# arancormonk/dsd-neo

Hardware: AMD Instinct MI355X
Metric: I/Q Msamples/s end-to-end (demod->FEC->MBE) per GPU; % HBM roofline (higher is better)
Workload: dtype f32

## Files before the change

### dsd-neo_amd/csrc/ddn_api_chain.cpp

```cpp
#include <hip/hip_runtime.h>
#include <hsa/hsa.h>
#include <hsa/hsa_ext_amd.h>

#include <condition_variable>
#include <cstdio>
#include <cstdlib>
#include <cstring>
#include <deque>
#include <mutex>
#include <new>
#include <thread>

#include "ddn_api_util.h"
#include "ddn_chain.h"
#include "ddn_device.h"
#include "ddn_hip.h"
#include "ddn_internal.h"
#include "ddn_mbe.h"

enum { NSET = 3 };
static inline int
set_prev(int cur) {
    return (cur + NSET - 1) % NSET;
}
// ... 666 lines not shown
        {
            std::unique_lock<std::mutex> lk(*c->out_mu);
            c->out_cv->wait(lk, [&] { return c->out_stop || !c->out_q->empty(); });
            if (c->out_stop) {
                return;
            }
            job = c->out_q->front();
            c->out_q->pop_front();
        }
        int rc = DDN_OK;
        if (hipEventSynchronize(c->ev_consumed[job.set]) != hipSuccess) {
            rc = DDN_EHIP;
        } else {
            rc = chain_copy_out(c, &job.out, job.set);
        }
        {
            std::lock_guard<std::mutex> lk(*c->out_mu);
            if (rc != DDN_OK && c->out_rc == DDN_OK) {
                c->out_rc = rc;
                snprintf(c->out_err, sizeof(c->out_err), "%s", ddn_last_error());
            }
            c->out_issued[job.set]++;
        }
        c->out_cv->notify_all();
    }
}

static int
out_worker_start(ddn_p25_chain* c) {
    if (c->out_thread) {
        return DDN_OK;
    }
    HIP_TRY(hipGetDevice(&c->out_dev));
    c->out_mu = new (std::nothrow) std::mutex();
    c->out_cv = new (std::nothrow) std::condition_variable();
    c->out_q = new (std::nothrow) std::deque<ddn_p25_chain::OutJob>();
    if (!c->out_mu || !c->out_cv || !c->out_q) {
        return DDN_ENOMEM;
    }
    c->out_thread = new (std::nothrow) std::thread(out_worker, c);
    return c->out_thread ? DDN_OK : DDN_ENOMEM;
}

static int
chain_issue_pending(ddn_p25_chain* c, hipEvent_t beside) {
    if (!c->have_pending) {
        return DDN_OK;
    }
    const int set = c->pending_set;
    if (c->sdma > 0) {
        DDN_TRY(out_worker_start(c));
        c->have_pending = 0;
        {
            std::lock_guard<std::mutex> lk(*c->out_mu);
            ddn_p25_chain::OutJob job;
            job.set = set;
            job.out = c->pending_out;
            c->out_q->push_back(job);
            c->out_submitted[set]++;
        }
        c->out_cv->notify_all();
        return out_take_rc(c);
    }
    HIP_TRY(hipStreamWaitEvent(c->s_copy2, c->ev_consumed[set], 0));
    if (beside) {
        HIP_TRY(hipStreamWaitEvent(c->s_copy2, beside, 0));
    }
    DDN_TRY(chain_copy_out(c, &c->pending_out, set));
    HIP_TRY(hipEventRecord(c->ev_out[set], c->s_copy2));
    c->have_pending = 0;
    return DDN_OK;
}

static int chain_issue_deferred(ddn_p25_chain* c, hipEvent_t gate);

static int
chain_settle_pending(ddn_p25_chain* c, hipStream_t st, bool deferred_too = true) {
    if (c->have_deferred && deferred_too) {
        const int set = c->deferred_set;
        DDN_TRY(chain_issue_deferred(c, nullptr));
        HIP_TRY(hipStreamWaitEvent(st, c->ev_consumed[set], 0));
    }
    if (!c->have_pending) {
        return DDN_OK;
    }
    const int set = c->pending_set;
    DDN_TRY(chain_issue_pending(c, nullptr));
    if (c->sdma > 0) {
        for (int k = 0; k < NSET; k++) {
            sdma_wait(c, k);
        }
        return DDN_OK;
    }
    HIP_TRY(hipStreamWaitEvent(st, c->ev_out[set], 0));
    return DDN_OK;
}

static int
chain_long_pdu(ddn_p25_chain* c, int cur, int flush, hipStream_t st) {
    const DdnLongPdu* lp = &c->lp;
    const int NW = lp->B * lp->W;
    const int32_t *d_ns = nullptr, *d_sp = nullptr;
    DDN_TRY(ddn_p25p1_framer_device_syncs(c->fr, &d_ns, &d_sp));
    HIP_TRY(ddn_dev_lpdu_index(lp, c->d_evl[cur], c->d_evdl[cur], c->d_nevl[cur], c->EL, d_sp, d_ns, c->d_nid[cur], c->d_cnt_full[cur],
                               c->stride, c->d_new[set_prev(cur)], c->step > 0 ? 1 : 0, flush, c->F, c->T, c->off97[0], st));
    HIP_TRY(ddn_dev_lpdu_gather(lp, c->d_rec[cur], c->d_cnt_full[cur], c->stride, st));
    HIP_TRY(ddn_dev_p25_half_rate_list_wanted_wide(lp->wk_llr, NW, 8, lp->wk_want, (uint32_t*)lp->wk_cand, lp->wk_cnt, st));
    HIP_TRY(ddn_dev_chain_pdu_take_first(lp->wk_cand, lp->wk_cnt, NW, lp->wk_b12, lp->wk_metric, st));
    DDN_TRY(ddn_fec_p25_mbf34_list_batch(lp->wk_llr, (size_t)NW, 8, lp->wk_want34, (ddn_p25_mbf34_candidate*)lp->wk_cand, lp->wk_cnt, st));
    HIP_TRY(ddn_dev_chain_pdu_r34_select(lp->wk_cand, lp->wk_cnt, lp->wk_want34, NW, lp->wk_b18, lp->wk_c9, st));
    HIP_TRY(ddn_dev_lpdu_scatter(lp, st));
    HIP_TRY(ddn_dev_lpdu_finish(lp, st));
    return DDN_OK;
}

static int
chain_decode(ddn_p25_chain* c, int cur, int flush, hipStream_t st, hipEvent_t ev_pre = nullptr, bool defer_synth = false) {
    const size_t S = c->S, V = c->V, stride = c->stride;
    const uint8_t* rec = c->d_rec[cur];
    if (c->timing) {
        HIP_TRY(hipEventRecord(c->ev_t[3], st));
    }
    HIP_TRY(ddn_dev_chain_counts(c->d_new[cur], c->T, c->B, flush, c->d_cnt_scan, c->d_cnt_full[cur], st));
    DDN_TRY(ddn_p25p1_framer_index(c->fr, c->d_fl[cur], c->d_cnt_scan, stride, st));
    {
        const int prev = set_prev(cur);
        HIP_TRY(ddn_dev_chain_events(c->d_evl[prev], c->d_evdl[prev], c->d_nevl[prev], c->d_new[prev], c->step > 0 ? 1 : 0, c->d_ev[cur],
                                     c->d_evd[cur], c->d_nev[cur], c->E, c->EL, c->T, c->B, c->d_evl[cur], c->d_evdl[cur], c->d_nevl[cur],
                                     st));
        const int32_t *d_ns = nullptr, *d_sp = nullptr;
        DDN_TRY(ddn_p25p1_framer_device_syncs(c->fr, &d_ns, &d_sp));
        HIP_TRY(ddn_dev_zero_words(c->d_list_n, 8, st));
        HIP_TRY(ddn_dev_chain_frames(c->d_evl[cur], c->d_evdl[cur], c->d_nevl[cur], c->EL, d_sp, d_ns, c->B, c->F, c->off97[0],
                                     c->off97[1], c->off97[2], c->d_nid[cur], c->d_tsbk[cur], c->d_tsbk_crc, c->d_cls, c->d_lists, c->d_list_n,
                                     st));
    }
    hipStream_t vst = st;
    if (!c->timing && st == c->s_aux) {
        HIP_TRY(hipEventRecord(c->ev_fork, st));
        HIP_TRY(hipStreamWaitEvent(c->s_voice, c->ev_fork, 0));
        vst = c->s_voice;
    }
    struct SelGuard {
        ~SelGuard() { ddn_sel_clear(); }
    } sel_guard;
    for (int i = 0; i < 2; i++) {
        const int ldu = i + 1;
        ddn_sel_set(c->d_lists + (size_t)i * S, c->d_list_n + i);
        DDN_TRY(ddn_p25p1_framer_gather_ldu_words(c->fr, ldu, rec, c->d_cnt_full[cur], stride, c->d_words[i], c->d_wrel, c->d_vldu, st));
        DDN_TRY(ddn_fec_hamming_10_6_3_batch(c->d_words[i], S * 24, c->d_werrs, st));
        DDN_TRY(ddn_p25p1_framer_pack_ldu_rs(c->fr, ldu, c->d_words[i], c->d_rs_d[i], c->d_rs_p[i], st));
        DDN_TRY(ddn_fec_p25_rs_batch(i == 0 ? DDN_RS_24_12_13 : DDN_RS_24_16_9, c->d_rs_d[i], c->d_rs_p[i], S, c->d_rs_st[i], st));
    }
    ddn_sel_set(c->d_lists + (size_t)DDN_LIST_HDU * S, c->d_list_n + DDN_LIST_HDU);
    DDN_TRY(ddn_p25p1_framer_gather_hdu(c->fr, rec, c->d_cnt_full[cur], stride, c->d_hdu_hex, c->d_hdu_par, nullptr, nullptr, c->d_vldu, st));
    DDN_TRY(ddn_fec_golay24_batch(6, c->d_hdu_hex, c->d_hdu_par, S * 36, c->d_hdu_st, nullptr, st));
    DDN_TRY(ddn_p25p1_framer_pack_hdu_rs(c->fr, c->d_hdu_hex, c->d_hdu_d, c->d_hdu_p, st));
    DDN_TRY(ddn_fec_p25_rs_batch(DDN_RS_36_20_17, c->d_hdu_d, c->d_hdu_p, S, c->d_hdu_rs, st));
    ddn_sel_set(c->d_lists + (size_t)DDN_LIST_TDULC * S, c->d_list_n + DDN_LIST_TDULC);
    DDN_TRY(ddn_p25p1_framer_gather_tdulc(c->fr, rec, c->d_cnt_full[cur], stride, c->d_td_d, c->d_td_p, nullptr, nullptr, c->d_vldu, st));
    DDN_TRY(ddn_fec_golay24_batch(12, c->d_td_d, c->d_td_p, S * 12, c->d_td_st, nullptr, st));
    DDN_TRY(ddn_p25p1_framer_pack_tdulc_rs(c->fr, c->d_td_d, c->d_td_rd, c->d_td_rp, st));
    DDN_TRY(ddn_fec_p25_rs_batch(DDN_RS_24_12_13, c->d_td_rd, c->d_td_rp, S, c->d_td_rs, st));
    ddn_sel_set(c->d_lists + (size_t)DDN_LIST_LSD * S, c->d_list_n + DDN_LIST_LSD);
    DDN_TRY(ddn_p25p1_framer_gather_lsd(c->fr, rec, c->d_cnt_full[cur], stride, c->d_lsd, c->d_lsd_llr, c->d_vldu, st));
    DDN_TRY(ddn_fec_p25_lsd_batch(c->d_lsd, c->d_lsd_llr, S * 2, c->d_lsd_ok, st));
    ddn_sel_clear();
    {
        const int32_t *d_ns = nullptr, *d_sp = nullptr;
        DDN_TRY(ddn_p25p1_framer_device_syncs(c->fr, &d_ns, &d_sp));
        const size_t NE = (size_t)c->B * (size_t)c->PF, NB = NE * (size_t)c->PB;
        HIP_TRY(ddn_dev_chain_pdu_index(c->d_evl[cur], c->d_evdl[cur], c->d_nevl[cur], c->EL, d_sp, d_ns, c->d_nid[cur], c->B, c->F, c->off97[0],
                                        c->PF, c->d_pdu_slot, c->d_pdu_hdr, c->d_pdu_info, c->d_n_pdu, st));
        HIP_TRY(ddn_dev_chain_pdu_gather(rec, c->d_cnt_full[cur], stride, d_sp, c->d_pdu_slot, c->d_pdu_info, c->B, c->F, c->PF, c->PB,
                                         c->d_pdu_llr, c->d_pdu_valid, st));
        HIP_TRY(ddn_dev_p25_half_rate_list_wanted(c->d_pdu_llr, (int)NB, 8, c->d_pdu_valid, (uint32_t*)c->d_pdu_cand, c->d_pdu_cnt, st));
        HIP_TRY(ddn_dev_chain_pdu_take_first(c->d_pdu_cand, c->d_pdu_cnt, (int)NB, c->d_pdu_blocks, c->d_pdu_metric, st));
        HIP_TRY(ddn_dev_chain_pdu_r34_wanted(c->d_pdu_slot, c->d_pdu_hdr, c->d_pdu_info, c->d_pdu_valid, (int)NB, c->PB, c->d_pdu_wanted, st));
        DDN_TRY(ddn_fec_p25_mbf34_list_batch(c->d_pdu_llr, NB, 8, c->d_pdu_wanted, (ddn_p25_mbf34_candidate*)c->d_pdu_cand, c->d_pdu_cnt, st));
        HIP_TRY(ddn_dev_chain_pdu_r34_select(c->d_pdu_cand, c->d_pdu_cnt, c->d_pdu_wanted, (int)NB, c->d_pdu_blocks18, c->d_pdu_crc9, st));
        HIP_TRY(ddn_dev_chain_pdu_combine(rec, c->d_cnt_full[cur], stride, d_sp, c->d_pdu_slot, c->d_pdu_info, c->d_pdu_llr, c->d_pdu_valid,
                                          c->d_pdu_blocks, (int)NE, c->PF, c->PB, c->d_pdu_hllr, c->d_pdu_wanted, st));
        HIP_TRY(ddn_dev_p25_half_rate_list_wanted(c->d_pdu_hllr, (int)NE, 8, c->d_pdu_wanted, (uint32_t*)c->d_pdu_cand, c->d_pdu_cnt, st));
        HIP_TRY(ddn_dev_chain_pdu_finish(c->d_pdu_slot, c->d_pdu_blocks, c->d_pdu_valid, c->d_pdu_blocks18, c->d_pdu_cand, c->d_pdu_cnt,
                                         c->d_pdu_wanted, (int)NE, c->PB, c->d_pdu_hdr, c->d_pdu_info, st));
    }
    if (c->lp.MB > 0) {
        DDN_TRY(chain_long_pdu(c, cur, flush, st));
    }
    if (c->timing) {
        HIP_TRY(hipEventRecord(c->ev_t[4], st));
    }
    if (c->want_rec2) {
        HIP_TRY(ddn_dev_chain_pack2(c->d_rec[cur], c->d_fl[cur], (size_t)c->B * c->stride, c->d_rec2[cur], vst));
        c->want_rec2 = 0;
    }
    DDN_TRY(ddn_p25p1_framer_voice_live(c->fr, c->d_nid[cur], c->d_cnt_full[cur], c->Fv, stride, c->d_first, c->d_sc, c->d_nldu, c->d_live_off,
                                        c->d_nlive[cur], vst));
    {
        const DdnVoiceLive a = chain_voice_live_args(c, cur);
        HIP_TRY(ddn_dev_voice_live_fill(&a, vst));
    }
    DDN_TRY(ddn_p25p1_imbe_deinterleave_live(rec, (size_t)c->B * stride, c->d_first, c->d_sc, V, c->d_live[cur], c->d_nlive[cur], c->d_imbe_fr,
                                             c->d_imbe_soft, c->d_imbe_fl, c->d_sc_out, vst));
    DDN_TRY(ddn_mbe_frame_decode_live(c->d_imbe_fr, c->d_imbe_fl, V, c->d_live[cur], c->d_nlive[cur], c->d_imbe_d, c->d_imbe_res, vst));
    if (ev_pre) {
        if (vst != st) {
            HIP_TRY(hipEventRecord(c->ev_join_a, vst));
            HIP_TRY(hipStreamWaitEvent(st, c->ev_join_a, 0));
        }
        HIP_TRY(hipEventRecord(ev_pre, st));
    }
    if (defer_synth && vst != st && ev_pre && c->cfg.vocoder) {
        DDN_TRY(ddn_mbe_params_only(c->mbe, c->d_imbe_d, c->d_imbe_res, (size_t)c->Fv * 9, c->d_nldu, c->d_res_out, vst));
        HIP_TRY(hipEventRecord(c->ev_join_a, vst));
        HIP_TRY(hipStreamWaitEvent(st, c->ev_join_a, 0));
        HIP_TRY(hipEventRecord(ev_pre, st));
        c->have_deferred = 1;
        c->deferred_set = cur;
        c->deferred_dense = 0;
        return DDN_OK;
    }
    if (c->cfg.vocoder) {
        DDN_TRY(ddn_mbe_synth_batch_live(c->mbe, c->d_imbe_d, c->d_imbe_res, (size_t)c->Fv * 9, c->d_nldu, c->d_live[cur], c->d_nlive[cur],
                                         c->d_pcm[cur], c->d_res_out, vst));
    }
    if (vst != st) {
        HIP_TRY(hipEventRecord(c->ev_join, vst));
        HIP_TRY(hipStreamWaitEvent(st, c->ev_join, 0));
    }
    if (c->timing) {
        HIP_TRY(hipEventRecord(c->ev_t[5], st));
    }
    return DDN_OK;
}

static int
chain_issue_deferred(ddn_p25_chain* c, hipEvent_t gate) {
    if (!c->have_deferred) {
        return DDN_OK;
    }
    const int set = c->deferred_set;
    c->have_deferred = 0;
    HIP_TRY(hipStreamWaitEvent(c->s_voice, c->ev_pre[set], 0));
    if (gate) {
        HIP_TRY(hipStreamWaitEvent(c->s_voice, gate, 0));
    }
    if (c->cfg.vocoder) {
        DDN_TRY(ddn_mbe_synth_only(c->mbe, (size_t)c->Fv * 9, c->d_live[set], c->d_nlive[set], c->d_pcm[set], c->s_voice));
        if (c->deferred_dense) {
            const size_t V = c->V;
            HIP_TRY(ddn_dev_chain_pcm_compact(c->d_imbe_res, c->d_pcm[set], (int)V, (long)V, c->d_pcm_bcnt, c->d_pcm_boff, c->d_pcm_dense[set],
                                              c->d_pcm_slot[set], c->d_pcm_total[set], c->s_voice));
        }
    }
    HIP_TRY(hipStreamWaitEvent(c->s_voice, c->ev_aux_done[set], 0));
    HIP_TRY(hipEventRecord(c->ev_consumed[set], c->s_voice));
    return DDN_OK;
}

extern "C" int
ddn_p25_chain_set_timing(ddn_p25_chain* c, int enable) {
    if (!c) {
        return DDN_EINVAL;
    }
    c->timing = enable ? 1 : 0;
    return DDN_OK;
}

extern "C" int
ddn_p25_chain_set_first_channel(ddn_p25_chain* c, int first) {
    if (!c || first < 0) {
        return DDN_EINVAL;
    }
    if (!c->mbe) {
        return DDN_OK;
    }
    const int rc = ddn_mbe_batch_set_first_stream(c->mbe, (uint32_t)first, nullptr);
    return rc != DDN_OK ? rc : (hipDeviceSynchronize() == hipSuccess ? DDN_OK : DDN_EHIP);
}

extern "C" int
ddn_p25_chain_get_stage_ms(ddn_p25_chain* c, float out4[4]) {
    if (!c || !out4) {
        return DDN_EINVAL;
    }
    DDN_TRY(ddn_p25_chain_wait(c));
    HIP_TRY(hipEventSynchronize(c->ev_t[5]));
    HIP_TRY(hipEventElapsedTime(&out4[0], c->ev_t[0], c->ev_t[1]));
    HIP_TRY(hipEventElapsedTime(&out4[1], c->ev_t[1], c->ev_t[2]));
    HIP_TRY(hipEventElapsedTime(&out4[2], c->ev_t[3], c->ev_t[4]));
    HIP_TRY(hipEventElapsedTime(&out4[3], c->ev_t[4], c->ev_t[5]));
    return DDN_OK;
}

extern "C" int
ddn_p25_chain_run(ddn_p25_chain* c, const void* d_iq, void* hip_stream) {
    if (!c || !d_iq) {
        return DDN_EINVAL;
    }
    c->after_flush = 0;
    hipStream_t st = (hipStream_t)hip_stream;
    DDN_TRY(chain_settle_pending(c, st));
    const int cur = (int)(c->step % NSET);
    DDN_TRY(chain_receive(c, d_iq, cur, st));
    DDN_TRY(chain_decode(c, cur, 0, st));
    HIP_TRY(hipEventRecord(c->ev_user, st));
    c->have_user_stream = 1;
    c->last_set = cur;
    c->step++;
    return DDN_OK;
}

extern "C" int
ddn_p25_chain_stage(ddn_p25_chain* c, int stage, const void* d_iq, void* hip_stream) {
    if (!c || stage < 0 || stage > 2 || (stage == 0 && !d_iq)) {
        return DDN_EINVAL;
    }
    c->after_flush = 0;
// ... 431 lines not shown
```

### dsd-neo_amd/csrc/ddn_block.hip

```cpp

#include <hip/hip_runtime.h>
#include <stdint.h>

#include <stdlib.h>
#include "ddn_bcode_dev.h"
#include "ddn_crc_dev.h"
#include "ddn_device.h"
#include "ddn_nid_dev.h"

using namespace ddn_nid;

__global__ __launch_bounds__(64) void
k_nid_decode(const uint8_t* __restrict__ bits63, const uint8_t* __restrict__ rel63, const int32_t* __restrict__ obs_nac,
             const uint8_t* __restrict__ parity, const uint8_t* __restrict__ parity_rel, int threshold, int n,
             int32_t* __restrict__ out4, int32_t* __restrict__ chase_list, int32_t* __restrict__ chase_count) {
    __shared__ uint8_t ex[128];
    __shared__ uint8_t lg[64];
    __shared__ uint8_t work[(23 + 24 + 24 + 24) * 64];
    gf_fill_wg(ex, lg);
    const Gf gf = {ex, lg};
    const Work wk = {work + threadIdx.x, work + 23 * 64 + threadIdx.x, work + 47 * 64 + threadIdx.x,
                     work + 71 * 64 + threadIdx.x};
    const int c = blockIdx.x * blockDim.x + threadIdx.x;
    if (c >= n) {
// ... 173 lines not shown
#pragma unroll
    for (int off = 32; off >= 1; off >>= 1) {
        const uint32_t o = __shfl_xor(m, off);
        m = o < m ? o : m;
    }
    if (m != 0xFFFFFFFFu && best_key == m) {
        int32_t* o = out4 + (size_t)c * 4;
        o[0] = best_dec.status;
        o[1] = best_dec.nac;
        o[2] = best_dec.duid;
        o[3] = best_dec.errs;
    }
}

__global__ __launch_bounds__(64) void
k_nid_wave(const uint8_t* __restrict__ bits63, const uint8_t* __restrict__ rel63, const int32_t* __restrict__ obs_nac,
           const uint8_t* __restrict__ parity, const uint8_t* __restrict__ parity_rel, int threshold, int n,
           int32_t* __restrict__ out4) {
    __shared__ uint8_t ex[128];
    __shared__ uint8_t lg[64];
    __shared__ uint8_t work[(23 + 24 + 24 + 24) * 64];
    __shared__ uint8_t masks[96];
    __shared__ uint8_t relb[64];
    const int lane = threadIdx.x;
    if (lane == 0) {
        chase_masks_fill(masks);
    }
    const int c = blockIdx.x;
    const uint8_t* bp = bits63 + (size_t)c * 63;
    const uint64_t w = __ballot(lane < 63 && bp[lane < 63 ? lane : 0] != 0);
    relb[lane] = (rel63 && lane < 63) ? rel63[(size_t)c * 63 + lane] : 0;
    gf_fill_wg(ex, lg);
    const Gf gf = {ex, lg};
    const Work wk = {work + lane, work + 23 * 64 + lane, work + 47 * 64 + lane, work + 71 * 64 + lane};
    const int par = parity ? (parity[c] ? 1 : 0) : 0;
    const int prel = parity_rel ? parity_rel[c] : 0;
    const int obs = obs_nac ? obs_nac[c] : 0;
    const NidRes r = nid_decode_wave(gf, wk, w, rel63 ? relb : nullptr, par, prel, obs, threshold, masks, lane);
    if (lane == 0) {
        int32_t* o = out4 + (size_t)c * 4;
        o[0] = r.status;
        o[1] = r.nac;
        o[2] = r.duid;
        o[3] = r.errs;
    }
}

static int
nid_wave_max() {
    static int v = -1;
    if (v < 0) {
        const char* e = DDN_EXP_ENV("DDN_NID_WAVE_MAX");
        const long x = e ? strtol(e, nullptr, 10) : 16384;
        v = (x < 0 || x > (1 << 24)) ? 16384 : (int)x;
    }
    return v;
}

extern "C" hipError_t
ddn_dev_nid_decode(const uint8_t* bits63, const uint8_t* rel63, const int32_t* obs_nac, const uint8_t* parity,
                   const uint8_t* parity_rel, int threshold, int n, int32_t* out4, hipStream_t st) {
    if (n <= 0) {
        return hipSuccess;
    }
    if (n <= nid_wave_max()) {
        hipLaunchKernelGGL(k_nid_wave, dim3((unsigned)n), dim3(64), 0, st, bits63, rel63, obs_nac, parity, parity_rel, threshold, n,
                           out4);
        return hipGetLastError();
    }
    int32_t* scratch = nullptr;
    int32_t *list = nullptr, *count = nullptr;
    if (rel63) {
        hipError_t e = hipMallocAsync((void**)&scratch, sizeof(int32_t) * ((size_t)n + 1), st);
        if (e != hipSuccess) {
            return e;
        }
        count = scratch;
        list = scratch + 1;
        e = hipMemsetAsync(count, 0, sizeof(int32_t), st);
        if (e != hipSuccess) {
            (void)hipFreeAsync(scratch, st);
            return e;
        }
    }
    hipLaunchKernelGGL(k_nid_decode, dim3((unsigned)((n + 63) / 64)), dim3(64), 0, st, bits63, rel63, obs_nac, parity,
                       parity_rel, threshold, n, out4, list, count);
    hipError_t e = hipGetLastError();
    if (e != hipSuccess || !rel63) {
        if (scratch) {
            (void)hipFreeAsync(scratch, st);
        }
        return e;
    }
    hipLaunchKernelGGL(k_nid_chase, dim3((unsigned)n), dim3(64), 0, st, bits63, rel63, obs_nac, parity, parity_rel,
                       threshold, (const int32_t*)list, (const int32_t*)count, out4);
    e = hipGetLastError();
    const hipError_t ef = hipFreeAsync(scratch, st);
    return e != hipSuccess ? e : ef;
}

extern "C" hipError_t
ddn_dev_hamming_10_6_3(uint8_t* bits10, int n, uint8_t* errs, hipStream_t st) {
    if (n <= 0) {
        return hipSuccess;
    }
    const DdnSel sel = ddn_sel_for(24);
    hipLaunchKernelGGL(k_hamming_10_6_3, dim3(ddn_sel_grid(&sel, ((unsigned long)n + DDN_WG - 1) / DDN_WG)), dim3(DDN_WG), 0, st, bits10, n, errs, sel);
    return hipGetLastError();
}

namespace {
__device__ __forceinline__ int
lsd_parity_of(int data) {
    int v = data << 8;
#pragma unroll
    for (int i = 15; i >= 8; i--) {
        if (v & (1 << i)) {
            v ^= 0x139 << (i - 8);
        }
    }
    return v & 0xFF;
}

__device__ __forceinline__ int
lsd_hard(int word) {
    const int data = (word >> 8) & 0xFF, parity = word & 0xFF;
    const int synd = parity ^ lsd_parity_of(data);
    if (synd == 0) {
        return word;
    }
    if ((synd & (synd - 1)) == 0) {
        return word ^ synd;
    }
#pragma unroll
    for (int pos = 0; pos < 8; pos++) {
        if (lsd_parity_of(1 << (7 - pos)) == synd) {
            return word ^ (1 << (15 - pos));
        }
    }
    return -1;
}

__global__ void
k_p25_lsd(uint8_t* __restrict__ bits16, const int16_t* __restrict__ llr16, int n, uint8_t* __restrict__ ok, DdnSel sel) {
    auto one = [&](long i) {
    uint8_t* b = bits16 + (size_t)i * 16;
    int word = 0;
    for (int k = 0; k < 16; k++) {
        word = (word << 1) | (b[k] & 1);
    }
    int fixed = lsd_hard(word);
    if (fixed < 0 && llr16) {
        const int16_t* l = llr16 + (size_t)i * 16;
        int cand[6], rel[6], nc = 0;
        unsigned taken = 0;
        for (int c = 0; c < 6; c++) {
            int bi = -1, br = 1 << 30;
            for (int k = 0; k < 16; k++) {
                const int r = l[k] < 0 ? -(int)l[k] : (int)l[k];
                if (r < 64 && !(taken & (1u << k)) && r < br) {
                    br = r;
                    bi = k;
                }
            }
            if (bi < 0) {
                break;
            }
            taken |= 1u << bi;
            cand[nc] = bi;
            rel[nc] = br;
            nc++;
        }
        int best = -1, best_pen = 999999;
        for (int mask = 1; mask < (1 << nc); mask++) {
            int w = word, pen = 0;
            for (int c = 0; c < nc; c++) {
                if (mask & (1 << c)) {
                    w ^= 1 << (15 - cand[c]);
                    pen += rel[c];
                }
            }
            if (pen >= best_pen) {
                continue;
            }
            const int f = lsd_hard(w);
            if (f >= 0) {
                best = f;
                best_pen = pen;
            }
        }
        fixed = best;
    }
    if (fixed >= 0) {
        for (int k = 0; k < 16; k++) {
            b[k] = (uint8_t)((fixed >> (15 - k)) & 1);
        }
    }
    ok[i] = fixed >= 0 ? 1 : 0;
    };
    ddn_sel_for_each(sel, (long)n, one);
}
}

extern "C" hipError_t
ddn_dev_p25_lsd(uint8_t* bits16, const int16_t* llr16, int n, uint8_t* ok, hipStream_t st) {
    if (n <= 0) {
        return hipSuccess;
    }
    const DdnSel sel = ddn_sel_for(2);
    hipLaunchKernelGGL(k_p25_lsd, dim3(ddn_sel_grid(&sel, ((unsigned long)n + DDN_WG - 1) / DDN_WG)), dim3(DDN_WG), 0, st, bits16, llr16, n, ok, sel);
    return hipGetLastError();
}

namespace {
__global__ void
k_p25_crc16(const uint8_t* __restrict__ bytes, int item_bytes, int n, uint8_t* __restrict__ ok) {
    const int i = blockIdx.x * blockDim.x + threadIdx.x;
    if (i >= n) {
        return;
    }
    const uint8_t* b = bytes + (size_t)i * item_bytes;
    const unsigned crc = ddn_crc::of_bytes(ddn_crc::CCITT16, b, item_bytes - 2);
    ok[i] = crc == (((unsigned)b[item_bytes - 2] << 8) | b[item_bytes - 1]) ? 1 : 0;
}
}

extern "C" hipError_t
ddn_dev_p25_crc16(const uint8_t* bytes, int item_bytes, int n, uint8_t* ok, hipStream_t st) {
    if (n <= 0) {
        return hipSuccess;
    }
    hipLaunchKernelGGL(k_p25_crc16, dim3((unsigned)((n + 255) / 256)), dim3(256), 0, st, bytes, item_bytes, n, ok);
    return hipGetLastError();
}
```

### dsd-neo_amd/csrc/ddn_mbe.hip

```cpp

#include <hip/hip_runtime.h>
#include <stdint.h>

#include "ddn_bcode_dev.h"
#include "ddn_device.h"
#include "ddn_mbe.h"
#include "ddn_mbe_dev.h"
#include "ddn_mbe_math.h"

namespace {

using Golay23 = ddn_bcode::Golay23<ddn_bcode::Golay23Msb>;

__device__ __forceinline__ uint32_t
golay_fix(uint32_t w, const uint32_t* tab, int& errs) {
    const uint32_t e = tab[ddn_bcode::Golay23Msb::syndrome(w)] & 0x7FF800u;
    errs = __popc(e);
    return w ^ e;
}

__device__ __forceinline__ uint32_t
hamming_fix(uint32_t w, int& errs) {
    const uint32_t syn = (uint32_t)ddn_bcode::syndrome(ddn_bcode::MBE_HAMMING_15_11, w);
    errs = 0;
    if (syn) {
        errs = 1;
#pragma unroll
        for (int p = 0; p < 15; p++) {
            if ((uint32_t)ddn_bcode::syndrome(ddn_bcode::MBE_HAMMING_15_11, 1u << p) == syn) {
                w ^= 1u << p;
            }
        }
    }
    return w;
}

#define DDN_MBE_FRAMES_PER_WG 32
template <int CODEC>
__device__ __forceinline__ void
frame_decode_lane(const uint8_t* f, uint8_t* o, int32_t* r5, bool soft_input) {
    constexpr int OB = CODEC == DDN_MBE_IMBE_7200X4400 ? 88 : 49;
    constexpr int ROWLEN = CODEC == DDN_MBE_IMBE_7200X4400 ? 23 : 24;
    const uint32_t* tab = Golay23::v.e;
    {
        uint32_t row[8];
        bool bad = false;
        constexpr int NROW = CODEC == DDN_MBE_IMBE_7200X4400 ? 8 : 4;
#pragma unroll
        for (int r = 0; r < NROW; r++) {
            uint32_t w = 0;
            for (int j = 0; j < ROWLEN; j++) {
                const uint32_t v = f[r * ROWLEN + j];
                bad |= v > 1u;
                w |= (v & 1u) << j;
            }
            row[r] = w;
        }
        int c0 = 0, c4 = 0, total = 0, e = 0;
        unsigned flags = MBE_PROCESS_FLAG_C0_VALID | (soft_input ? MBE_PROCESS_FLAG_SOFT_INPUT : 0u);
        if (CODEC == DDN_MBE_IMBE_7200X4400) {
            flags |= MBE_PROCESS_FLAG_C4_VALID;
            row[0] = golay_fix(row[0], tab, c0);
            total = c0;
            uint32_t pr = (16u * (row[0] >> 11)) & 0xFFFFu;
#pragma unroll
            for (int r = 1; r < 7; r++) {
                const int len = r < 4 ? 23 : 15;
                uint32_t mask = 0;
                for (int j = len - 1; j >= 0; j--) {
                    pr = (173u * pr + 13849u) & 0xFFFFu;
                    mask |= (pr >> 15) << j;
                }
                row[r] ^= mask;
            }
#pragma unroll
            for (int r = 1; r < 4; r++) {
                row[r] = golay_fix(row[r], tab, e);
                total += e;
            }
#pragma unroll
            for (int r = 4; r < 7; r++) {
                row[r] = hamming_fix(row[r] & 0x7FFFu, e);
                if (r == 4) {
                    c4 = e;
                }
                total += e;
            }
            int k = 0;
#pragma unroll
            for (int r = 0; r < 4; r++) {
                for (int j = 22; j > 10; j--) {
                    o[k++] = (uint8_t)((row[r] >> j) & 1u);
                }
            }
#pragma unroll
            for (int r = 4; r < 7; r++) {
                for (int j = 14; j >= 4; j--) {
                    o[k++] = (uint8_t)((row[r] >> j) & 1u);
                }
            }
            for (int j = 6; j >= 0; j--) {
                o[k++] = (uint8_t)((row[7] >> j) & 1u);
            }
        } else {
            uint32_t w0 = golay_fix(row[0] >> 1, tab, c0);
            row[0] = (w0 << 1) | (row[0] & 1u);
            uint32_t pr = (16u * (w0 >> 11)) & 0xFFFFu;
            uint32_t mask = 0;
            for (int j = 22; j >= 0; j--) {
                pr = (173u * pr + 13849u) & 0xFFFFu;
                mask |= (pr >> 15) << j;
            }
            row[1] = golay_fix((row[1] ^ mask) & 0x7FFFFFu, tab, e);
            total = c0 + e;
            int k = 0;
            for (int j = 23; j > 11; j--) {
                o[k++] = (uint8_t)((row[0] >> j) & 1u);
            }
            for (int j = 22; j > 10; j--) {
                o[k++] = (uint8_t)((row[1] >> j) & 1u);
            }
            for (int j = 10; j >= 0; j--) {
                o[k++] = (uint8_t)((row[2] >> j) & 1u);
            }
            for (int j = 13; j >= 0; j--) {
                o[k++] = (uint8_t)((row[3] >> j) & 1u);
            }
        }
        if (bad) {
            for (int k = 0; k < OB; k++) {
                o[k] = 0;
            }
            r5[0] = (int32_t)DDN_MBE_RESULT_INVALID;
            r5[1] = r5[2] = r5[3] = r5[4] = 0;
        } else {
            r5[0] = (int32_t)flags;
            r5[1] = c0;
            r5[2] = c4;
            r5[3] = total;
            r5[4] = total - c0;
        }
    }
}

template <int CODEC>
__global__ __launch_bounds__(64) void
k_mbe_frame_decode(const uint8_t* __restrict__ frames, const uint8_t* __restrict__ soft, size_t n,
                   uint8_t* __restrict__ bits_out, int32_t* __restrict__ result) {
    constexpr int FB = CODEC == DDN_MBE_IMBE_7200X4400 ? 184 : 96;
    constexpr int OB = CODEC == DDN_MBE_IMBE_7200X4400 ? 88 : 49;
    constexpr int FPW = DDN_MBE_FRAMES_PER_WG;
    __shared__ uint8_t stage[FPW * FB];
    __shared__ uint8_t outb[FPW * OB];
    const int lane = threadIdx.x;
    const size_t f0 = (size_t)blockIdx.x * FPW;
    const size_t nf = (n - f0) < (size_t)FPW ? (n - f0) : (size_t)FPW;
    const uint8_t* src = frames + f0 * FB;
    for (size_t i = lane; i < nf * FB; i += 64) {
        stage[i] = src[i];
    }
    __syncthreads();
    if ((size_t)lane < nf) {
        frame_decode_lane<CODEC>(stage + lane * FB, outb + lane * OB, result + (f0 + lane) * 5, soft != nullptr);
    }
    __syncthreads();
    uint8_t* dst = bits_out + f0 * OB;
    for (size_t i = lane; i < nf * OB; i += 64) {
        dst[i] = outb[i];
    }
}

__global__ __launch_bounds__(64) __attribute__((amdgpu_waves_per_eu(3))) void
k_mbe_frame_decode_live(const uint8_t* __restrict__ frames, int n_slots, const int32_t* __restrict__ live_slot,
                        const int32_t* __restrict__ n_live, uint8_t* __restrict__ bits_out, int32_t* __restrict__ result) {
    constexpr int FB = 184, OB = 88, FPW = DDN_MBE_FRAMES_PER_WG;
    __shared__ uint8_t stage[FPW * FB];
    __shared__ uint8_t outb[FPW * OB];
    int n = *n_live;
    n = n < n_slots ? n : n_slots;
    auto slot_of = [&](int i) {
        const int v = live_slot[i];
        return (size_t)(v < 0 ? 0 : (v >= n_slots ? n_slots - 1 : v));
    };
    for (int i0 = blockIdx.x * FPW; i0 < n; i0 += gridDim.x * FPW) {
        int lane = threadIdx.x;
        asm volatile("" : "+v"(lane));
        const int nf = (n - i0) < FPW ? (n - i0) : FPW;
        int mine = (int)slot_of(i0 + (lane < nf ? lane : nf - 1));
        for (int k = 0; k < nf; k++) {
            const uint8_t* src = frames + (size_t)__shfl(mine, k) * FB;
            for (int b = lane; b < FB; b += 64) {
                stage[k * FB + b] = src[b];
            }
        }
        __syncthreads();
        if (lane < nf) {
            frame_decode_lane<DDN_MBE_IMBE_7200X4400>(stage + lane * FB, outb + lane * OB, reinterpret_cast<int32_t*>(stage + lane * FB), false);
        }
        __syncthreads();
        asm volatile("" : "+v"(lane));
        mine = (int)slot_of(i0 + (lane < nf ? lane : nf - 1));
        for (int k = 0; k < nf; k++) {
            const size_t v = (size_t)__shfl(mine, k);
            uint8_t* dst = bits_out + v * OB;
            for (int b = lane; b < OB; b += 64) {
                dst[b] = outb[k * OB + b];
            }
            if (lane < 5) {
                result[v * 5 + lane] = reinterpret_cast<const int32_t*>(stage + k * FB)[lane];
            }
        }
        __syncthreads();
    }
}

struct LaneParms {
    float w0, gamma;
    int L, K, repeat;
    int V;
    float Ml, log2Ml, PHI, PSI;
};

__device__ __forceinline__ LaneParms
lane_init(int l) {
    LaneParms p;
    p.w0 = 0.09378f;
    p.gamma = 0.0f;
    p.L = 30;
    p.K = 10;
    p.repeat = 0;
    p.V = 0;
    p.Ml = 0.0f;
    p.log2Ml = 0.0f;
    p.PHI = 0.0f;
    p.PSI = MBE_PI_F / 2.0f;
    (void)l;
    return p;
}

__device__ __forceinline__ LaneParms
lane_load(const mbe_parms* s, int l) {
    LaneParms p;
    const int i = l <= 56 ? l : 56;
    p.w0 = s->w0;
    p.gamma = s->gamma;
    p.L = s->L;
    p.K = s->K;
    p.repeat = s->repeat;
    p.V = s->Vl[i];
    p.Ml = s->Ml[i];
    p.log2Ml = s->log2Ml[i];
    p.PHI = s->PHIl[i];
    p.PSI = s->PSIl[i];
    return p;
}

__device__ __forceinline__ void
lane_store(mbe_parms* s, const LaneParms& p, int l, int un) {
    if (l == 0) {
        s->w0 = p.w0;
        s->gamma = p.gamma;
        s->L = p.L;
        s->K = p.K;
        s->repeat = p.repeat;
        s->un = un;
    }
    if (l <= 56) {
        s->Vl[l] = p.V;
        s->Ml[l] = p.Ml;
        s->log2Ml[l] = p.log2Ml;
        s->PHIl[l] = p.PHI;
        s->PSIl[l] = p.PSI;
    }
}

__device__ __forceinline__ float
dequant(uint32_t b, int bits, float step) {
    if (bits <= 0) {
        return 0.0f;
    }
    return step * (((float)b - (float)(1u << (bits - 1))) + 0.5f);
}

__device__ __forceinline__ float
idct_term(const float* C, int J, int j) {
    float acc = 0.0f;
    for (int k = 1; k <= J; k++) {
        const float a = (k == 1) ? 1.0f : 2.0f;
        const float ang = (MBE_PI_F * (float)(k - 1) * ((float)j - 0.5f)) / (float)J;
        acc = acc + (a * C[k]) * mbe_cosf(ang);
    }
    return acc;
}

template <int CODEC>
__global__ __launch_bounds__(64) void
k_mbe_params(const uint8_t* __restrict__ bits, const int32_t* __restrict__ res_in, int n_frames,
             const ddn_mbe_tables* __restrict__ T, const float* __restrict__ half_log2, DdnMbeStream* __restrict__ streams,
             int tail_rule, DdnMbeFrameRec* __restrict__ recs, int32_t* __restrict__ res_out, const int32_t* __restrict__ n_ldu) {
    constexpr int NB = CODEC == DDN_MBE_IMBE_7200X4400 ? 88 : 49;
    __shared__ uint32_t fld[64];
    __shared__ float sG[12], sR[12], sC[64], sPl[64], sA[64], sB[64];
    __shared__ float sCb[5][64];
    const int s = blockIdx.x;
    const int l = threadIdx.x;
    const int n_walk = n_ldu ? (9 * n_ldu[s] < n_frames ? 9 * n_ldu[s] : n_frames) : n_frames;
    if (n_walk <= 0) {
        return;
    }
    DdnMbeStream* st = streams + s;
    LaneParms cur = lane_load(&st->cur, l), prev = lane_load(&st->prev, l), enh = lane_load(&st->enh, l);
    uint32_t frame_no = st->frame_no;
    const uint32_t seed = st->seed;

    for (int f = 0; f < n_walk; f++) {
        const size_t fi = (size_t)s * (size_t)n_frames + (size_t)f;
        const uint8_t* d = bits + fi * NB;
        int32_t r[5] = {0, 0, 0, 0, 0};
        if (res_in) {
#pragma unroll
            for (int k = 0; k < 5; k++) {
                r[k] = res_in[fi * 5 + k];
            }
        }
        unsigned flags = (unsigned)r[0];
        const int errs2 = r[3];
        DdnMbeFrameRec* rec = recs + fi;
        const uint32_t v0 = (l < NB) ? d[l] : 0u, v1 = (l + 64 < NB) ? d[l + 64] : 0u;
        const unsigned long long m0 = __ballot(v0 & 1u), m1 = __ballot(v1 & 1u);
        const bool invalid = __any((v0 > 1u) || (v1 > 1u)) || (flags & DDN_MBE_RESULT_INVALID);
        auto bit = [&](int p) -> uint32_t { return (uint32_t)(((p < 64 ? m0 >> p : m1 >> (p - 64))) & 1ull); };
        bool skip = invalid;
        if (!skip && tail_rule && CODEC == DDN_MBE_IMBE_7200X4400 && errs2 >= 10) {
            uint32_t prefix = 0;
            for (int p = 0; p < 8; p++) {
                prefix = (prefix << 1) | bit(p);
            }
            const int set = __popcll(m0) + __popcll(m1 & 0xFFFFFFull);
            if (prefix == 0xFCu && set <= 24) {
                skip = true;
                flags = 0;
                r[1] = r[2] = r[3] = r[4] = 0;
            }
        }
        if (skip) {
            if (l == 0) {
                rec->flags = DDN_MBE_REC_SILENCE;
                rec->maxl = 0;
                if (res_out) {
                    res_out[fi * 5 + 0] = (int32_t)(invalid ? DDN_MBE_RESULT_INVALID : flags);
                    res_out[fi * 5 + 1] = r[1];
                    res_out[fi * 5 + 2] = r[2];
                    res_out[fi * 5 + 3] = r[3];
                    res_out[fi * 5 + 4] = r[4];
                }
            }
            continue;
        }

        cur.repeat = prev.repeat;
        int bad = 0;
        float Tl = 0.0f;
        float rho = 0.65f, extra = 0.0f;
        int L = 0;
        float unvc = 1.0f;
// ... 370 lines not shown
                    return (w * cM) * mbe_cosf((cw0l * (float)(n - 160)) + cP);
                }
                const float c3 = unvoiced_mix(cw0, cw0l, l, n, base, 0x200u);
                return (((c3 * MBE_UVSINE) * w) * cM) * MBE_QFACTOR;
            };
            const bool p_on = pM != 0.0f, c_on = cM != 0.0f;
            if (inA && p_on) {
                acc[0] = acc[0] + prev_side(nA, wpA);
            }
            if (inB && (p_on || c_on)) {
                acc[1] = acc[1] + ((p_on ? prev_side(nB, wpB) : 0.0f) + (c_on ? cur_side(nB, wcB) : 0.0f));
            }
            if (inC && c_on) {
                acc[2] = acc[2] + cur_side(nC, wcC);
            }
        }
    }
    if (lane < 56) {
        out[lane] = acc[0];
    }
    if (lane < 49) {
        out[56 + lane] = acc[1];
    }
    if (lane < 55) {
        out[105 + lane] = acc[2];
    }
}

__global__ __launch_bounds__(64) void
k_mbe_synth(const DdnMbeFrameRec* __restrict__ recs, float* __restrict__ pcm) {
    synth_frame(recs + blockIdx.x, pcm + (size_t)blockIdx.x * 160, threadIdx.x);
}

__global__ __launch_bounds__(64) void
k_mbe_synth_live(const DdnMbeFrameRec* __restrict__ recs, int n_slots, const int32_t* __restrict__ live_slot,
                 const int32_t* __restrict__ n_live, float* __restrict__ pcm) {
    int n = *n_live;
    n = n < n_slots ? n : n_slots;
    for (int i = blockIdx.x; i < n; i += gridDim.x) {
        int v = __builtin_amdgcn_readfirstlane(live_slot[i]);
        v = v < 0 ? 0 : (v >= n_slots ? n_slots - 1 : v);
        int lane = threadIdx.x;
        asm volatile("" : "+v"(lane));
        synth_frame(recs + v, pcm + (size_t)v * 160, lane);
    }
}

__global__ void
k_mbe_result_skip(const uint8_t* __restrict__ skip, size_t n, int32_t* __restrict__ result) {
    const size_t i = (size_t)blockIdx.x * blockDim.x + threadIdx.x;
    if (i < n && skip[i]) {
        result[i * 5] = (int32_t)((uint32_t)result[i * 5] | DDN_MBE_RESULT_INVALID);
    }
}

__global__ void
k_mbe_result_skip_live(const uint8_t* __restrict__ skip, int n_slots, const int32_t* __restrict__ live_slot,
                       const int32_t* __restrict__ n_live, int32_t* __restrict__ result) {
    int n = *n_live;
    n = n < n_slots ? n : n_slots;
    for (int i = blockIdx.x * blockDim.x + threadIdx.x; i < n; i += gridDim.x * blockDim.x) {
        int v = live_slot[i];
        v = v < 0 ? 0 : (v >= n_slots ? n_slots - 1 : v);
        if (skip[v]) {
            result[(size_t)v * 5] = (int32_t)((uint32_t)result[(size_t)v * 5] | DDN_MBE_RESULT_INVALID);
        }
    }
}

__global__ void
k_mbe_stream_init(DdnMbeStream* streams, int n, uint32_t seed0) {
    const int s = blockIdx.x;
    const int l = threadIdx.x;
    if (s >= n) {
        return;
    }
    const LaneParms p = lane_init(l);
    lane_store(&streams[s].cur, p, l, 0);
    lane_store(&streams[s].prev, p, l, 0);
    lane_store(&streams[s].enh, p, l, 0);
    if (l == 0) {
        streams[s].frame_no = 0;
        streams[s].seed = seed0 + (uint32_t)s;
    }
}
}

extern "C" hipError_t
ddn_dev_mbe_frame_decode(int codec, const uint8_t* frames, const uint8_t* soft, size_t n, uint8_t* bits, int32_t* result,
                         hipStream_t st) {
    if (n == 0) {
        return hipSuccess;
    }
    const dim3 grid((unsigned)((n + DDN_MBE_FRAMES_PER_WG - 1) / DDN_MBE_FRAMES_PER_WG)), blk(64);
    if (codec == DDN_MBE_IMBE_7200X4400) {
        hipLaunchKernelGGL(k_mbe_frame_decode<DDN_MBE_IMBE_7200X4400>, grid, blk, 0, st, frames, soft, n, bits, result);
    } else {
        hipLaunchKernelGGL(k_mbe_frame_decode<DDN_MBE_AMBE_3600X2450>, grid, blk, 0, st, frames, soft, n, bits, result);
    }
    return hipGetLastError();
}

extern "C" hipError_t
ddn_dev_mbe_stream_init(DdnMbeStream* streams, int n_streams, uint32_t seed0, hipStream_t st) {
    if (n_streams <= 0) {
        return hipSuccess;
    }
    hipLaunchKernelGGL(k_mbe_stream_init, dim3((unsigned)n_streams), dim3(64), 0, st, streams, n_streams, seed0);
    return hipGetLastError();
}

extern "C" hipError_t
ddn_dev_mbe_params(int codec, const uint8_t* bits, const int32_t* res_in, int n_streams, int n_frames,
                   const ddn_mbe_tables* d_tables, const float* d_half_log2, DdnMbeStream* streams, int tail_rule,
                   DdnMbeFrameRec* recs, int32_t* res_out, const int32_t* n_ldu, hipStream_t st) {
    if (n_streams <= 0 || n_frames <= 0) {
        return hipSuccess;
    }
    const dim3 grid((unsigned)n_streams), blk(64);
    if (codec == DDN_MBE_IMBE_7200X4400) {
        hipLaunchKernelGGL(k_mbe_params<DDN_MBE_IMBE_7200X4400>, grid, blk, 0, st, bits, res_in, n_frames, d_tables,
                           d_half_log2, streams, tail_rule, recs, res_out, n_ldu);
    } else {
        hipLaunchKernelGGL(k_mbe_params<DDN_MBE_AMBE_3600X2450>, grid, blk, 0, st, bits, res_in, n_frames, d_tables,
                           d_half_log2, streams, tail_rule, recs, res_out, n_ldu);
    }
    return hipGetLastError();
}

extern "C" hipError_t
ddn_dev_mbe_synth(const DdnMbeFrameRec* recs, size_t n_frames_total, float* pcm, hipStream_t st) {
    if (n_frames_total == 0) {
        return hipSuccess;
    }
    hipLaunchKernelGGL(k_mbe_synth, dim3((unsigned)n_frames_total), dim3(64), 0, st, recs, pcm);
    return hipGetLastError();
}

extern "C" hipError_t
ddn_dev_mbe_result_skip(const uint8_t* skip, size_t n, int32_t* result, hipStream_t st) {
    if (n == 0) {
        return hipSuccess;
    }
    hipLaunchKernelGGL(k_mbe_result_skip, dim3((unsigned)((n + 63) / 64)), dim3(64), 0, st, skip, n, result);
    return hipGetLastError();
}

extern "C" hipError_t
ddn_dev_mbe_frame_decode_live(const uint8_t* frames, int n_slots, const int32_t* live_slot, const int32_t* n_live, uint8_t* bits,
                              int32_t* result, hipStream_t st) {
    if (n_slots <= 0) {
        return hipSuccess;
    }
    const int groups = (n_slots + DDN_MBE_FRAMES_PER_WG - 1) / DDN_MBE_FRAMES_PER_WG;
    const int grid = groups < DDN_VOICE_LIVE_GRID_DECODE ? groups : DDN_VOICE_LIVE_GRID_DECODE;
    hipLaunchKernelGGL(k_mbe_frame_decode_live, dim3((unsigned)grid), dim3(64), 0, st, frames, n_slots, live_slot, n_live, bits, result);
    return hipGetLastError();
}

extern "C" hipError_t
ddn_dev_mbe_result_skip_live(const uint8_t* skip, int n_slots, const int32_t* live_slot, const int32_t* n_live, int32_t* result,
                             hipStream_t st) {
    if (n_slots <= 0) {
        return hipSuccess;
    }
    const int groups = (n_slots + 63) / 64;
    const int grid = groups < DDN_VOICE_LIVE_GRID / 8 ? groups : DDN_VOICE_LIVE_GRID / 8;
    hipLaunchKernelGGL(k_mbe_result_skip_live, dim3((unsigned)grid), dim3(64), 0, st, skip, n_slots, live_slot, n_live, result);
    return hipGetLastError();
}

extern "C" hipError_t
ddn_dev_mbe_synth_live(const DdnMbeFrameRec* recs, int n_slots, const int32_t* live_slot, const int32_t* n_live, float* pcm,
                       hipStream_t st) {
    if (n_slots <= 0) {
        return hipSuccess;
    }
    const int grid = n_slots < DDN_VOICE_LIVE_GRID_SYNTH ? n_slots : DDN_VOICE_LIVE_GRID_SYNTH;
    hipLaunchKernelGGL(k_mbe_synth_live, dim3((unsigned)grid), dim3(64), 0, st, recs, n_slots, live_slot, n_live, pcm);
    return hipGetLastError();
}
```

Measured before the change: 27310.

## Vectorize MBE frame bit packing and decode live frames directly per lane

The MBE frame decoder now reads the input frame as 32-bit words and packs bits using multiply tricks instead of byte-by-byte loops. Output bits are assembled in registers and written as 32-bit words. The live decode kernel drops shared-memory staging and the grid-stride loop and maps one lane to one frame, launching multiple chunks from the host. The LSD gather and decode move earlier in the FEC sequence, and the LSD chase candidates are kept in packed integers instead of local arrays. The new code requires 8-byte aligned buffers, and reading frames directly per lane may give less coalesced global access than the old staging.

Result: no change. 27470 (median of 6 runs) (+0.6%).

```diff
diff --git a/dsd-neo_amd/csrc/ddn_api_chain.cpp b/dsd-neo_amd/csrc/ddn_api_chain.cpp
--- a/dsd-neo_amd/csrc/ddn_api_chain.cpp
+++ b/dsd-neo_amd/csrc/ddn_api_chain.cpp
@@ -842,6 +842,9 @@
         DDN_TRY(ddn_p25p1_framer_pack_ldu_rs(c->fr, ldu, c->d_words[i], c->d_rs_d[i], c->d_rs_p[i], st));
         DDN_TRY(ddn_fec_p25_rs_batch(i == 0 ? DDN_RS_24_12_13 : DDN_RS_24_16_9, c->d_rs_d[i], c->d_rs_p[i], S, c->d_rs_st[i], st));
     }
+    ddn_sel_set(c->d_lists + (size_t)DDN_LIST_LSD * S, c->d_list_n + DDN_LIST_LSD);
+    DDN_TRY(ddn_p25p1_framer_gather_lsd(c->fr, rec, c->d_cnt_full[cur], stride, c->d_lsd, c->d_lsd_llr, c->d_vldu, st));
+    DDN_TRY(ddn_fec_p25_lsd_batch(c->d_lsd, c->d_lsd_llr, S * 2, c->d_lsd_ok, st));
     ddn_sel_set(c->d_lists + (size_t)DDN_LIST_HDU * S, c->d_list_n + DDN_LIST_HDU);
     DDN_TRY(ddn_p25p1_framer_gather_hdu(c->fr, rec, c->d_cnt_full[cur], stride, c->d_hdu_hex, c->d_hdu_par, nullptr, nullptr, c->d_vldu, st));
     DDN_TRY(ddn_fec_golay24_batch(6, c->d_hdu_hex, c->d_hdu_par, S * 36, c->d_hdu_st, nullptr, st));
@@ -852,9 +855,6 @@
     DDN_TRY(ddn_fec_golay24_batch(12, c->d_td_d, c->d_td_p, S * 12, c->d_td_st, nullptr, st));
     DDN_TRY(ddn_p25p1_framer_pack_tdulc_rs(c->fr, c->d_td_d, c->d_td_rd, c->d_td_rp, st));
     DDN_TRY(ddn_fec_p25_rs_batch(DDN_RS_24_12_13, c->d_td_rd, c->d_td_rp, S, c->d_td_rs, st));
-    ddn_sel_set(c->d_lists + (size_t)DDN_LIST_LSD * S, c->d_list_n + DDN_LIST_LSD);
-    DDN_TRY(ddn_p25p1_framer_gather_lsd(c->fr, rec, c->d_cnt_full[cur], stride, c->d_lsd, c->d_lsd_llr, c->d_vldu, st));
-    DDN_TRY(ddn_fec_p25_lsd_batch(c->d_lsd, c->d_lsd_llr, S * 2, c->d_lsd_ok, st));
     ddn_sel_clear();
     {
         const int32_t *d_ns = nullptr, *d_sp = nullptr;
diff --git a/dsd-neo_amd/csrc/ddn_block.hip b/dsd-neo_amd/csrc/ddn_block.hip
--- a/dsd-neo_amd/csrc/ddn_block.hip
+++ b/dsd-neo_amd/csrc/ddn_block.hip
@@ -349,7 +349,9 @@
     int fixed = lsd_hard(word);
     if (fixed < 0 && llr16) {
         const int16_t* l = llr16 + (size_t)i * 16;
-        int cand[6], rel[6], nc = 0;
+        unsigned cand = 0;
+        unsigned long long rel = 0;
+        int nc = 0;
         unsigned taken = 0;
         for (int c = 0; c < 6; c++) {
             int bi = -1, br = 1 << 30;
@@ -364,8 +366,8 @@
                 break;
             }
             taken |= 1u << bi;
-            cand[nc] = bi;
-            rel[nc] = br;
+            cand |= (unsigned)bi << (4 * nc);
+            rel |= (unsigned long long)br << (6 * nc);
             nc++;
         }
         int best = -1, best_pen = 999999;
@@ -373,8 +375,8 @@
             int w = word, pen = 0;
             for (int c = 0; c < nc; c++) {
                 if (mask & (1 << c)) {
-                    w ^= 1 << (15 - cand[c]);
-                    pen += rel[c];
+                    w ^= 1 << (15 - (int)((cand >> (4 * c)) & 15u));
+                    pen += (int)((rel >> (6 * c)) & 63ull);
                 }
             }
             if (pen >= best_pen) {
diff --git a/dsd-neo_amd/csrc/ddn_mbe.hip b/dsd-neo_amd/csrc/ddn_mbe.hip
--- a/dsd-neo_amd/csrc/ddn_mbe.hip
+++ b/dsd-neo_amd/csrc/ddn_mbe.hip
@@ -46,16 +46,30 @@
         uint32_t row[8];
         bool bad = false;
         constexpr int NROW = CODEC == DDN_MBE_IMBE_7200X4400 ? 8 : 4;
+        constexpr int NW = NROW * ROWLEN / 4;
+        static_assert(NROW * ROWLEN % 8 == 0 && NW <= 46, "frame bytes in whole 8-byte words");
+        uint32_t sb[(NW + 7) / 8 + 1] = {};
+        uint32_t over = 0;
+        const uint32_t* fw = reinterpret_cast<const uint32_t*>(f);
+#pragma unroll
+        for (int i = 0; i < NW; i++) {
+            const uint32_t w = fw[i];
+            over |= w & 0xFEFEFEFEu;
+            sb[i / 8] |= (((w & 0x01010101u) * 0x01020408u) >> 24) << (4 * (i % 8));
+        }
+        bad = over != 0;
 #pragma unroll
         for (int r = 0; r < NROW; r++) {
-            uint32_t w = 0;
-            for (int j = 0; j < ROWLEN; j++) {
-                const uint32_t v = f[r * ROWLEN + j];
-                bad |= v > 1u;
-                w |= (v & 1u) << j;
-            }
-            row[r] = w;
-        }
+            const int p = r * ROWLEN, q = p / 32, sh = p % 32;
+            const uint64_t two = ((uint64_t)sb[q + 1] << 32) | sb[q];
+            row[r] = (uint32_t)(two >> sh) & ((1u << ROWLEN) - 1u);
+        }
+        uint32_t ob[(OB + 31) / 32 + 1] = {};
+        auto put = [&](int at, uint32_t field, int n) {
+            const uint64_t v = (uint64_t)(__brev(field) >> (32 - n)) << (at % 32);
+            ob[at / 32] |= (uint32_t)v;
+            ob[at / 32 + 1] |= (uint32_t)(v >> 32);
+        };
         int c0 = 0, c4 = 0, total = 0, e = 0;
         unsigned flags = MBE_PROCESS_FLAG_C0_VALID | (soft_input ? MBE_PROCESS_FLAG_SOFT_INPUT : 0u);
         if (CODEC == DDN_MBE_IMBE_7200X4400) {
@@ -86,22 +100,15 @@
                 }
                 total += e;
             }
-            int k = 0;
 #pragma unroll
             for (int r = 0; r < 4; r++) {
-                for (int j = 22; j > 10; j--) {
-                    o[k++] = (uint8_t)((row[r] >> j) & 1u);
-                }
+                put(12 * r, row[r] >> 11, 12);
             }
 #pragma unroll
             for (int r = 4; r < 7; r++) {
-                for (int j = 14; j >= 4; j--) {
-                    o[k++] = (uint8_t)((row[r] >> j) & 1u);
-                }
-            }
-            for (int j = 6; j >= 0; j--) {
-                o[k++] = (uint8_t)((row[7] >> j) & 1u);
-            }
+                put(48 + 11 * (r - 4), row[r] >> 4, 11);
+            }
+            put(81, row[7], 7);
         } else {
             uint32_t w0 = golay_fix(row[0] >> 1, tab, c0);
             row[0] = (w0 << 1) | (row[0] & 1u);
@@ -113,24 +120,30 @@
             }
             row[1] = golay_fix((row[1] ^ mask) & 0x7FFFFFu, tab, e);
             total = c0 + e;
-            int k = 0;
-            for (int j = 23; j > 11; j--) {
-                o[k++] = (uint8_t)((row[0] >> j) & 1u);
-            }
-            for (int j = 22; j > 10; j--) {
-                o[k++] = (uint8_t)((row[1] >> j) & 1u);
-            }
-            for (int j = 10; j >= 0; j--) {
-                o[k++] = (uint8_t)((row[2] >> j) & 1u);
-            }
-            for (int j = 13; j >= 0; j--) {
-                o[k++] = (uint8_t)((row[3] >> j) & 1u);
-            }
+            put(0, row[0] >> 12, 12);
+            put(12, row[1] >> 11, 12);
+            put(24, row[2], 11);
+            put(35, row[3], 14);
         }
         if (bad) {
+#pragma unroll
+            for (int k = 0; k < (OB + 31) / 32 + 1; k++) {
+                ob[k] = 0;
+            }
+        }
+        if (OB % 4 == 0) {
+            uint32_t* ow = reinterpret_cast<uint32_t*>(o);
+#pragma unroll
+            for (int i = 0; i < OB / 4; i++) {
+                ow[i] = (((ob[i / 8] >> (4 * (i % 8))) & 15u) * 0x00204081u) & 0x01010101u;
+            }
+        } else {
+#pragma unroll
             for (int k = 0; k < OB; k++) {
-                o[k] = 0;
-            }
+                o[k] = (uint8_t)((ob[k / 32] >> (k % 32)) & 1u);
+            }
+        }
+        if (bad) {
             r5[0] = (int32_t)DDN_MBE_RESULT_INVALID;
             r5[1] = r5[2] = r5[3] = r5[4] = 0;
         } else {
@@ -150,8 +163,8 @@
     constexpr int FB = CODEC == DDN_MBE_IMBE_7200X4400 ? 184 : 96;
     constexpr int OB = CODEC == DDN_MBE_IMBE_7200X4400 ? 88 : 49;
     constexpr int FPW = DDN_MBE_FRAMES_PER_WG;
-    __shared__ uint8_t stage[FPW * FB];
-    __shared__ uint8_t outb[FPW * OB];
+    __shared__ __attribute__((aligned(8))) uint8_t stage[FPW * FB];
+    __shared__ __attribute__((aligned(8))) uint8_t outb[FPW * OB];
     const int lane = threadIdx.x;
     const size_t f0 = (size_t)blockIdx.x * FPW;
     const size_t nf = (n - f0) < (size_t)FPW ? (n - f0) : (size_t)FPW;
@@ -170,47 +183,19 @@
     }
 }
 
-__global__ __launch_bounds__(64) __attribute__((amdgpu_waves_per_eu(3))) void
-k_mbe_frame_decode_live(const uint8_t* __restrict__ frames, int n_slots, const int32_t* __restrict__ live_slot,
+__global__ __launch_bounds__(64) void
+k_mbe_frame_decode_live(const uint8_t* __restrict__ frames, int n_slots, int i0, const int32_t* __restrict__ live_slot,
                         const int32_t* __restrict__ n_live, uint8_t* __restrict__ bits_out, int32_t* __restrict__ result) {
-    constexpr int FB = 184, OB = 88, FPW = DDN_MBE_FRAMES_PER_WG;
-    __shared__ uint8_t stage[FPW * FB];
-    __shared__ uint8_t outb[FPW * OB];
+    constexpr int FB = 184, OB = 88;
     int n = *n_live;
     n = n < n_slots ? n : n_slots;
-    auto slot_of = [&](int i) {
-        const int v = live_slot[i];
-        return (size_t)(v < 0 ? 0 : (v >= n_slots ? n_slots - 1 : v));
-    };
-    for (int i0 = blockIdx.x * FPW; i0 < n; i0 += gridDim.x * FPW) {
-        int lane = threadIdx.x;
-        asm volatile("" : "+v"(lane));
-        const int nf = (n - i0) < FPW ? (n - i0) : FPW;
-        int mine = (int)slot_of(i0 + (lane < nf ? lane : nf - 1));
-        for (int k = 0; k < nf; k++) {
-            const uint8_t* src = frames + (size_t)__shfl(mine, k) * FB;
-            for (int b = lane; b < FB; b += 64) {
-                stage[k * FB + b] = src[b];
-            }
-        }
-        __syncthreads();
-        if (lane < nf) {
-            frame_decode_lane<DDN_MBE_IMBE_7200X4400>(stage + lane * FB, outb + lane * OB, reinterpret_cast<int32_t*>(stage + lane * FB), false);
-        }
-        __syncthreads();
-        asm volatile("" : "+v"(lane));
-        mine = (int)slot_of(i0 + (lane < nf ? lane : nf - 1));
-        for (int k = 0; k < nf; k++) {
-            const size_t v = (size_t)__shfl(mine, k);
-            uint8_t* dst = bits_out + v * OB;
-            for (int b = lane; b < OB; b += 64) {
-                dst[b] = outb[k * OB + b];
-            }
-            if (lane < 5) {
-                result[v * 5 + lane] = reinterpret_cast<const int32_t*>(stage + k * FB)[lane];
-            }
-        }
-        __syncthreads();
+    const int i = i0 + (int)blockIdx.x * 64 + (int)threadIdx.x;
+    if (i < n) {
+        int v = live_slot[i];
+        v = v < 0 ? 0 : (v >= n_slots ? n_slots - 1 : v);
+        const uint8_t* f = static_cast<const uint8_t*>(__builtin_assume_aligned(frames + (size_t)v * FB, 8));
+        uint8_t* o = static_cast<uint8_t*>(__builtin_assume_aligned(bits_out + (size_t)v * OB, 8));
+        frame_decode_lane<DDN_MBE_IMBE_7200X4400>(f, o, result + (size_t)v * 5, false);
     }
 }
 
@@ -887,9 +872,15 @@
     if (n_slots <= 0) {
         return hipSuccess;
     }
-    const int groups = (n_slots + DDN_MBE_FRAMES_PER_WG - 1) / DDN_MBE_FRAMES_PER_WG;
-    const int grid = groups < DDN_VOICE_LIVE_GRID_DECODE ? groups : DDN_VOICE_LIVE_GRID_DECODE;
-    hipLaunchKernelGGL(k_mbe_frame_decode_live, dim3((unsigned)grid), dim3(64), 0, st, frames, n_slots, live_slot, n_live, bits, result);
+    if (((uintptr_t)frames | (uintptr_t)bits) & 7u) {
+        return hipErrorInvalidValue;
+    }
+    const int groups = (n_slots + 63) / 64;
+    for (int g0 = 0; g0 < groups; g0 += DDN_VOICE_LIVE_GRID_DECODE) {
+        const int grid = groups - g0 < DDN_VOICE_LIVE_GRID_DECODE ? groups - g0 : DDN_VOICE_LIVE_GRID_DECODE;
+        hipLaunchKernelGGL(k_mbe_frame_decode_live, dim3((unsigned)grid), dim3(64), 0, st, frames, n_slots, g0 * 64, live_slot, n_live, bits,
+                           result);
+    }
     return hipGetLastError();
 }
 
```
